# bowman-lab/enspara

Measured on AMD Instinct MI355X. Metric: frame x center RMSD pairs/sec in k-centers assign, higher is better.
Workload: dtype f32

## Files before the change

enspara_amd/csrc/ek_api_run.hip:

```cpp
#include "ek_ctx.h"
#include "ek_run_policy.h"
#include "ek_view.h"
#include <cmath>

void ek_view_free(ek_ctx *c)
{
    (void)ek_dev_free(c->v_aos);
    (void)ek_dev_free(c->v_tiles);
    (void)ek_dev_free(c->v_qtiles);
    (void)ek_dev_free(c->v_G);
    (void)ek_dev_free(c->v_dist);
    (void)ek_dev_free(c->v_assign);
    (void)ek_dev_free(c->v_act);
    (void)ek_dev_free(c->v_blockcnt);
    (void)ek_dev_free(c->v_blockoff);
    (void)ek_dev_free(c->v_count);
    c->v_aos = c->v_tiles = c->v_qtiles = nullptr;
    c->v_G = nullptr;
    c->v_dist = nullptr;
    c->v_assign = nullptr;
    c->v_act = c->v_blockcnt = c->v_blockoff = c->v_count = nullptr;
    c->view_cap = 0;
}

static int ek_view_alloc(ek_ctx *c, int64_t frames)
{
    const int64_t cap = (frames + EK_TILE - 1) / EK_TILE * EK_TILE;
    if (c->view_cap >= cap)
        return EK_OK;
    EK_HIP(ek_wait(c));
    ek_view_free(c);
    const size_t nt = (size_t)(cap / EK_TILE), A3 = (size_t)3 * c->A;
    const size_t nblk = ek_view_sel_blocks(std::max<int64_t>(c->n, 1));
    hipError_t e = hipSuccess;
#define EK_VALLOC(ptr, bytes)                                                  \
    if (e == hipSuccess)                                                       \
        e = ek_malloc_named(c, (void **)&(ptr), (bytes), #ptr);
    EK_VALLOC(c->v_aos, (size_t)cap * A3 * sizeof(float));
    EK_VALLOC(c->v_tiles, nt * A3 * EK_TILE * sizeof(float));
    EK_VALLOC(c->v_qtiles, ek_quad_tiles_bytes((int64_t)nt, c->A));
    EK_VALLOC(c->v_G, (size_t)cap * sizeof(double));
    EK_VALLOC(c->v_dist, (size_t)cap * sizeof(float));
    EK_VALLOC(c->v_assign, (size_t)cap * sizeof(int32_t));
    EK_VALLOC(c->v_act, (size_t)cap * sizeof(uint32_t));
    EK_VALLOC(c->v_blockcnt, nblk * sizeof(uint32_t));
    EK_VALLOC(c->v_blockoff, nblk * sizeof(uint32_t));
    EK_VALLOC(c->v_count, 2 * sizeof(uint32_t));
    if (e == hipSuccess)
        e = hipMemsetAsync(c->v_count, 0, 2 * sizeof(uint32_t), c->stream);
#undef EK_VALLOC
    if (e != hipSuccess) {
        (void)hipGetLastError();
        ek_view_free(c);
        if (e == hipErrorOutOfMemory) {
            c->view_nomem = true;
            return EK_ENOMEM;
        }
        EK_HIP(e);
    }
    c->view_cap = cap;
    return EK_OK;
}

struct EkViewRun {
    bool on = false;
    int64_t n = 0;
    int32_t label_lo = 0;
    double guard = 0.0;
    bool tiles_valid = false;
};

static hipError_t ek_view_poison(ek_ctx *c)
{
    const size_t cap = (size_t)c->view_cap, nt = cap / EK_TILE, A3 = (size_t)3 * c->A;
    hipError_t e = hipMemsetAsync(c->v_aos, 0xFF, cap * A3 * sizeof(float), c->stream);
    if (e == hipSuccess)
        e = hipMemsetAsync(c->v_tiles, 0xFF, nt * A3 * EK_TILE * sizeof(float), c->stream);
    if (e == hipSuccess)
        e = hipMemsetAsync(c->v_qtiles, 0xFF, ek_quad_tiles_bytes((int64_t)nt, c->A),
                           c->stream);
    if (e == hipSuccess)
        e = hipMemsetAsync(c->v_G, 0xFF, cap * sizeof(double), c->stream);
    if (e == hipSuccess)
        e = hipMemsetAsync(c->v_dist, 0xFF, cap * sizeof(float), c->stream);
    if (e == hipSuccess)
        e = hipMemsetAsync(c->v_assign, 0xFF, cap * sizeof(int32_t), c->stream);
    return e;
}

static bool ek_view_build(ek_ctx *c, int64_t n_v)
{
    ek_launch_view_build(c->v_act, n_v, c->A, c->qt_valid, c->aos, c->G, c->dist, c->assign,
                         c->v_aos, c->qt_valid ? c->v_qtiles : c->v_tiles, c->v_G, c->v_dist,
                         c->v_assign, c->stream);
    return !c->qt_valid;
}

static void ek_view_scatter_back(ek_ctx *c, EkViewRun &v)
{
    ek_launch_view_scatter(c->v_act, v.n, c->v_dist, c->v_assign, c->dist, c->assign,
                           c->hist, v.label_lo, c->hist_cap, c->ctl, c->goff, c->stream);
    v.on = false;
}

void ek_round_of(ek_ctx *c, int T, double cutoff, EkRound &R)
{
    R.dist = c->dist;
    R.assign = c->assign;
    R.vecs = c->vecs;
    R.n = c->n;
    R.n_pad = c->n_pad;
    R.goff = c->goff;
    R.A = c->A;
    R.T = T;
    R.tiles = c->tiles;
    R.qtiles = c->qtiles;
    R.aos = c->aos;
    R.G = c->G;
    R.recs = c->recsT;
    R.plan = c->plan;
    R.pend = c->pend;
    R.ord = c->ord;
    R.blockmax = c->blockmax;
    R.pm = c->pm;
    R.fm = c->fine_pick ? c->fm : nullptr;
    R.sweep = (c->pass_sweep == 2 ||
               (c->pass_sweep == 1 && ek_sweep_pays(c->n))) ? 1 : 0;
    R.top = c->top;
    R.ctile = c->ctile;
    R.ctrace = c->ctrace;
    R.hist = c->hist;
    R.ctl = c->ctl;
// ... 86 lines not shown
    if (!c->ti_tmask)
        EK_HIP(ek_dev_malloc((void **)&c->ti_tmask,
                         (size_t)std::max<int64_t>(c->n_tiles, 1) * sizeof(uint32_t)));
    return EK_OK;
}

static void ek_run_use_store(EkRun &run, bool the_view)
{
    ek_ctx *c = run.c;
    EkRound &R = run.R;
    if (the_view) {
        R.dist = c->v_dist;
        R.assign = c->v_assign;
        R.tiles = c->v_tiles;
        R.qtiles = c->v_qtiles;
        R.aos = c->v_aos;
        R.G = c->v_G;
        R.n = run.view.n;
        R.n_pad = (run.view.n + EK_TILE - 1) / EK_TILE * EK_TILE;
    } else {
        R.dist = c->dist;
        R.assign = c->assign;
        R.tiles = c->tiles;
        R.qtiles = c->qtiles;
        R.aos = c->aos;
        R.G = c->G;
        R.n = c->n;
        R.n_pad = c->n_pad;
    }
    run.nb = (int)((R.n + EK_BLOCK - 1) / EK_BLOCK);
    R.sweep = (run.fused && (c->pass_sweep == 2 ||
                             (c->pass_sweep == 1 && ek_sweep_pays(R.n)))) ? 1 : 0;
    R.cutoff = the_view ? std::max(run.dist_cutoff, run.view.guard) : run.dist_cutoff;
}

static void ek_run_leave_view(EkRun &run)
{
    if (run.pending) {
        ek_launch_round_flush(run.R, run.c->stream);
        run.pending = false;
// ... 8 lines not shown
    EkViewRun &view = run.view;
    run.looked = false;
    const EkViewPlan p =
        run.vp.decide(run.cr.last_max, run.rho, run.shrink, run.look_cnt,
                      view.on ? view.n : 0, c->n, left, run.per_round, run.forced);
    if (!p.build)
        return EK_OK;
    if (view.on) {
        ek_run_leave_view(run);
    } else if (run.pending) {
        ek_launch_round_flush(run.R, c->stream);
        run.pending = false;
    }
    uint32_t nv = 0;
    ek_launch_view_select(c->dist, c->n, p.theta, c->v_blockcnt, c->v_blockoff, c->v_act,
                          c->view_cap, c->v_count, c->stream);
    EK_CHECK_LAUNCH();
    EK_HIP(hipMemcpyAsync(&nv, c->v_count, sizeof(nv), hipMemcpyDeviceToHost, c->stream));
    EK_HIP(ek_wait(c));
    if (nv > 0 && (int64_t)nv < c->n && (int64_t)nv <= c->view_cap) {
        view.n = nv;
        view.label_lo = run.cr.n_done;
        view.guard = p.guard;
        if (run.view_mode == 3)
            EK_HIP(ek_view_poison(c));
        view.tiles_valid = ek_view_build(c, view.n);
        EK_CHECK_LAUNCH();
        view.on = true;
        ek_run_use_store(run, true);
        EK_HIP(hipMemsetAsync(c->vmask, 0, (size_t)(run.R.n_pad / EK_WAVE) * sizeof(uint32_t),
                              c->stream));
        c->view_stats[0]++;
    }
// ... 146 lines not shown
                     : ek_run_enqueue_unfused(run, form, batch);
}

static int ek_run_carry_look(EkRun &run)
{
    ek_ctx *c = run.c;
    if (!run.view_mode || run.vp.pause.tick())
        return EK_OK;
    const int64_t want_cap =
        run.forced ? c->n : (int64_t)std::ceil(run.shrink * (double)c->n);
    if (ek_view_alloc(c, want_cap) != EK_OK) {
        (void)hipGetLastError();
        run.view_mode = 0;
        return EK_OK;
    }
    EK_HIP(hipMemsetAsync(c->v_count, 0, sizeof(run.look_cnt), c->stream));
    ek_launch_view_look(run.R.dist, run.R.n, c->ctl, run.rho, EK_VIEW_REL, EK_VIEW_ABS,
                        c->v_count, c->stream);
    if (run.view.on)
        ek_launch_view_look(c->dist, c->n, c->ctl, run.rho, EK_VIEW_REL, EK_VIEW_ABS,
                            c->v_count + 1, c->stream);
    EK_CHECK_LAUNCH();
    EK_HIP(hipMemcpyAsync(run.look_cnt, c->v_count, sizeof(run.look_cnt),
                          hipMemcpyDeviceToHost, c->stream));
    run.looked = true;
    return EK_OK;
}

static int ek_run_read_back(EkRun &run, int form, int32_t &got, int32_t &ran)
{
    ek_ctx *c = run.c;
    const bool one = form == 1, masks = run.R.tmask != nullptr;
    const int32_t before = run.cr.n_done;
    EK_HIP(hipMemcpyAsync(&run.cr, c->ctl, sizeof(run.cr), hipMemcpyDeviceToHost, c->stream));
    unsigned long long ti_now[2] = {0, 0};
    if (masks)
        EK_HIP(hipMemcpyAsync(ti_now, c->ti_stats, sizeof(ti_now), hipMemcpyDeviceToHost,
                              c->stream));
// ... 281 lines not shown
}

extern "C" int ek_view_layout_check(ek_ctx *c, float theta, int64_t *out)
{
    if (!c || !out)
        return ek_fail(EK_EARG, "ek_view_layout_check: NULL argument");
    if (!c->loaded || c->n <= 0)
        return ek_fail(EK_ESTATE, "ek_view_layout_check: no frames loaded");
    EK_HIP(hipSetDevice(c->device));
    out[0] = out[1] = out[2] = out[3] = 0;
    int rc = ek_view_alloc(c, c->n);
    if (rc)
        return rc;
    uint32_t nv = 0;
    ek_launch_view_select(c->dist, c->n, theta, c->v_blockcnt, c->v_blockoff, c->v_act,
                          c->view_cap, c->v_count, c->stream);
    EK_CHECK_LAUNCH();
    EK_HIP(hipMemcpyAsync(&nv, c->v_count, sizeof(nv), hipMemcpyDeviceToHost, c->stream));
    EK_HIP(ek_wait(c));
    out[0] = nv;
    if (nv == 0 || (int64_t)nv > c->view_cap)
        return EK_OK;
    const size_t nt = ((size_t)nv + EK_TILE - 1) / EK_TILE, A3 = (size_t)3 * c->A;
    const size_t tile_words = nt * A3 * EK_TILE;
    const size_t quad_bytes = ek_quad_tiles_bytes((int64_t)nt, c->A);
    float *r_aos = nullptr, *r_tiles = nullptr, *r_qtiles = nullptr, *r_dist = nullptr;
    double *r_G = nullptr;
    int32_t *r_assign = nullptr;
    unsigned long long *diff = nullptr, got[3] = {0, 0, 0};
    hipError_t e = ek_dev_malloc((void **)&r_aos, (size_t)nv * A3 * sizeof(float));
    if (e == hipSuccess)
        e = ek_dev_malloc((void **)&r_tiles, tile_words * sizeof(float));
    if (e == hipSuccess)
        e = ek_dev_malloc((void **)&r_qtiles, quad_bytes);
    if (e == hipSuccess)
        e = ek_dev_malloc((void **)&r_G, (size_t)nv * sizeof(double));
    if (e == hipSuccess)
        e = ek_dev_malloc((void **)&r_dist, (size_t)nv * sizeof(float));
    if (e == hipSuccess)
        e = ek_dev_malloc((void **)&r_assign, (size_t)nv * sizeof(int32_t));
    if (e == hipSuccess)
        e = ek_dev_malloc((void **)&diff, sizeof(got));
    if (e == hipSuccess)
        e = hipMemsetAsync(diff, 0, sizeof(got), c->stream);
    if (e == hipSuccess)
        e = ek_view_poison(c);
    if (e == hipSuccess) {
        ek_launch_view_gather(c->v_act, nv, c->A, c->aos, c->G, c->dist, c->assign, r_aos,
                              r_tiles, r_G, r_dist, r_assign, c->stream);
        ek_launch_quad_tiles(r_tiles, (int64_t)nt, c->A, r_qtiles, c->stream);
        if (!ek_view_build(c, nv))
            ek_launch_view_tiles(c->v_qtiles, (int64_t)nt, c->A, c->v_tiles, c->stream);
        if (c->qt_valid)
            ek_launch_view_diff(c->v_qtiles, r_qtiles, quad_bytes / 4, diff, c->stream);
        ek_launch_view_diff(c->v_tiles, r_tiles, tile_words, diff + 1, c->stream);
        ek_launch_view_diff(c->v_aos, r_aos, (size_t)nv * A3, diff + 2, c->stream);
        ek_launch_view_diff(c->v_G, r_G, (size_t)nv * 2, diff + 2, c->stream);
        ek_launch_view_diff(c->v_dist, r_dist, (size_t)nv, diff + 2, c->stream);
        ek_launch_view_diff(c->v_assign, r_assign, (size_t)nv, diff + 2, c->stream);
        e = hipGetLastError();
    }
    if (e == hipSuccess)
        e = hipMemcpyAsync(got, diff, sizeof(got), hipMemcpyDeviceToHost, c->stream);
    if (e == hipSuccess)
        e = ek_wait(c);
    else
        (void)hipStreamSynchronize(c->stream);
    (void)ek_dev_free(r_aos);
    (void)ek_dev_free(r_tiles);
    (void)ek_dev_free(r_qtiles);
    (void)ek_dev_free(r_G);
    (void)ek_dev_free(r_dist);
    (void)ek_dev_free(r_assign);
    (void)ek_dev_free(diff);
    EK_HIP(e);
    out[1] = (int64_t)got[0];
    out[2] = (int64_t)got[1];
    out[3] = (int64_t)got[2];
    return EK_OK;
}

extern "C" int ek_last_run_form(ek_ctx *c, int64_t *out)
{
// ... 16 lines not shown
```

enspara_amd/csrc/ek_common.h:

```cpp
#pragma once
#include <hip/hip_runtime.h>
#include <stdint.h>
#include <stddef.h>

#include "../../include/enspara_hip.h"
#include "ek_track.h"
#include "ek_pam_limits.h"

#define EK_BLOCK 256
#define EK_WAVE 64
#define EK_MAX_ATOMS 4096

struct EkRecHdr {
    float maxdist;
    int32_t valid;
    int64_t gidx;
    double trace;
    int64_t reserved;
};
static_assert(sizeof(EkRecHdr) == 32, "record header is 32 bytes");

static inline __host__ __device__ size_t ek_rec_bytes(int A)
{
    return (sizeof(EkRecHdr) + (size_t)12 * (size_t)A + 15) & ~(size_t)15;
// ... 86 lines not shown
    uint32_t *vmask = nullptr;
    const uint32_t *tmask = nullptr;
    EkBlockMax *sweep_pm = nullptr;
    EkBlockMax *sweep_fm = nullptr;
    int sweep_nb = 0;
};
struct EkRound {
    float *dist;
    int32_t *assign;
    float *vecs;
    int64_t n, n_pad, goff;
    int A, T;
    const float *tiles;
    const float *qtiles;
    const float *aos;
    const double *G;
    unsigned char *recs;
    EkPlan *plan;
    EkPend *pend;
    EkChainOrd *ord;
    EkBlockMax *blockmax;
    EkBlockMax *pm;
    EkBlockMax *fm;
    unsigned char *top;
    float *ctile;
    double *ctrace;
    EkHist *hist;
    EkCtl *ctl;
    EkChainRow *rows;
    uint32_t *vmask;
    unsigned int *tick;
    double cutoff;
    float *ti_tab = nullptr;
    uint32_t *tmask = nullptr;
    unsigned long long *ti_stats = nullptr;
    int pick_cap = 4;
    int sweep = 0;
};
void ek_launch_round_ti(const EkRound &r, int max_labels, hipStream_t s);
void ek_launch_round_pass(const EkRound &r, hipStream_t s, bool with_order = true);
void ek_launch_round_chain(const EkRound &r, int bootstrap, hipStream_t s);
void ek_launch_round_next(const EkRound &r, int bootstrap, hipStream_t s);
void ek_launch_round_flush(const EkRound &r, hipStream_t s);

#define EK_MS_MAX_WORLD 64
#ifndef EK_MS_SLOTS
#define EK_MS_SLOTS 128
#endif
struct EkMsMsg {
    int32_t n_recs;
    int32_t cn;
    int32_t state;
    int32_t pad;
// ... 312 lines not shown
```

enspara_amd/csrc/ek_ctx.h:

```cpp
#pragma once
#include "ek_common.h"
#include "ek_pam_sparse.h"
#include "ek_pam_policy.h"

#include <stdarg.h>
#include <stdio.h>
#include <stdlib.h>
#include <string.h>

#include <algorithm>
#include <condition_variable>
#include <mutex>
#include <new>
#include <thread>
#include <vector>

void ek_msm_scratch_free(void *w);

#define EK_N_FORMS 5

int ek_set_error(int code, const char *fmt, ...);
#define ek_fail ek_set_error

#define EK_HIP(call)                                                           \
// ... 280 lines not shown
    double *ctrace = nullptr;
    int chain = 1;
    int64_t n_pad = 0;
    int32_t last_passes = 0;
    int adapt = 1;
    int64_t st_rounds[EK_N_FORMS] = {0, 0, 0, 0, 0};
    int64_t st_centers[EK_N_FORMS] = {0, 0, 0, 0, 0};
    int64_t last_form[6] = {0, 0, 0, 0, 0, 0};
    hipEvent_t evb0 = nullptr, evb1 = nullptr;

    int active_view = 1;
    int view_rho = 750;
    int view_ratio = 800;
    bool view_nomem = false;
    int64_t view_cap = 0;
    float *v_aos = nullptr, *v_tiles = nullptr, *v_qtiles = nullptr;
    double *v_G = nullptr;
    float *v_dist = nullptr;
    int32_t *v_assign = nullptr;
    uint32_t *v_act = nullptr;
    uint32_t *v_blockcnt = nullptr, *v_blockoff = nullptr;
    uint32_t *v_count = nullptr;
    int64_t view_stats[4] = {0, 0, 0, 0};

    EkMsState *ms = nullptr;
    unsigned char *ms_mbox = nullptr;
    uint32_t *ms_flags = nullptr;
    EkMsXchg ms_x;
    int ms_peers = 0;
    std::vector<void *> ms_ipc;
    int ms_T = 0;
    int ms_small = 0;
    hipEvent_t ms_ev[4] = {nullptr, nullptr, nullptr, nullptr};
    double ms_t[3] = {0.0, 0.0, 0.0};
    int64_t ms_t_n = 0;
    EkMsState ms_last;

// ... 48 lines not shown
```

enspara_amd/csrc/ek_round.hip:

```cpp
#include "ek_common.h"
#include "ek_qcp.h"
#include "ek_reduce.h"
#include "ek_chain_dev.h"
#include "ek_top_dev.h"

#ifdef EK_ROUND_STAMPS
__device__ unsigned int ek_stamp_count;
#define EK_STAMP(k) if (threadIdx.x == 0) st[k] = __builtin_amdgcn_s_memrealtime()
#else
#define EK_STAMP(k)
#endif

#define EK_ROUND_THREADS 1024

template <int NV>
__global__ void __launch_bounds__(EK_ROUND_THREADS)
ek_round_chain_kernel(EkRound r, int bootstrap)
{
    constexpr int EK_ROUND_FPT = 4;
    __shared__ float sv[EK_MAX_CANDS];
    __shared__ uint32_t si[EK_MAX_CANDS];
    __shared__ int s_napply, s_fine;
    extern __shared__ uint32_t skip[];
    const int tid = threadIdx.x;
// ... 236 lines not shown
                   64 * (v[8] / v[0]), 10 * (v[9] / v[0]), 10 * (v[10] / (v[0] / 4)),
                   10 * (v[11] / (v[12] ? v[12] : 1)), v[12]);
            for (int k = 0; k < 64 * 16; ++k)
                t[k] = 0;
        }
    }
#endif
    const EkTop *top = (const EkTop *)r.top;
    const bool done = r.ctl->stopped || r.ctl->n_done >= r.ctl->limit;
    if (!done) {
        const int lane = tid & (EK_WAVE - 1);
        const int w = blockIdx.x * (EK_BLOCK / EK_WAVE) + tid / EK_WAVE;
        const int i = w / EK_LIST_M, j = w % EK_LIST_M;
        if (i < j && j < top->n) {
            const int A = r.A;
            const float *x = r.aos + (size_t)top->idx[i] * 3 * A;
            const float *y = r.aos + (size_t)top->idx[j] * 3 * A;
            float S[9] = {0.f, 0.f, 0.f, 0.f, 0.f, 0.f, 0.f, 0.f, 0.f};
            for (int a = lane; a < A; a += EK_WAVE) {
                const float x0 = x[3 * a], x1 = x[3 * a + 1], x2 = x[3 * a + 2];
                const float y0 = y[3 * a], y1 = y[3 * a + 1], y2 = y[3 * a + 2];
                S[0] += x0 * y0; S[1] += x0 * y1; S[2] += x0 * y2;
                S[3] += x1 * y0; S[4] += x1 * y1; S[5] += x1 * y2;
                S[6] += x2 * y0; S[7] += x2 * y1; S[8] += x2 * y2;
            }
#pragma unroll
            for (int q = 0; q < 9; ++q)
#pragma unroll
                for (int off = 32; off >= 1; off >>= 1)
                    S[q] += __shfl_xor(S[q], off, 64);
            if (lane == 0) {
                const float d = ek_rmsd_from_S(S, r.G[top->idx[i]],
// ... 103 lines not shown
            plan->maxdist[tid] = sval[sel[tid]];
            plan->trace[tid] = tr;
            r.ctrace[tid] = tr;
        } else {
            h->maxdist = -__builtin_inff();
            h->valid = 0;
            h->gidx = -1;
            h->trace = 0.0;
            h->reserved = 0;
            r.ctrace[tid] = 0.0;
        }
    }
    const int A3 = 3 * r.A;
    if (T >= 16 && tid == 0)
        r.plan->n_rec = ns;
    for (int k0 = 0; T < 16 && k0 * EK_BLOCK < A3; k0 += 4) {
        float v[T][4];
#pragma unroll
        for (int c = 0; c < T; ++c) {
            const float *src = r.aos + (size_t)sidx[sel[c < ns ? c : 0]] * A3;
#pragma unroll
            for (int u = 0; u < 4; ++u) {
                const int row = tid + (k0 + u) * EK_BLOCK;
                v[c][u] = (c < ns && row < A3) ? src[row] : 0.f;
            }
        }
#pragma unroll
        for (int c = 0; c < T; ++c) {
            float *rec = (float *)(r.recs + (size_t)c * rstride + sizeof(EkRecHdr));
#pragma unroll
            for (int u = 0; u < 4; ++u) {
                const int row = tid + (k0 + u) * EK_BLOCK;
                if (row >= A3)
                    continue;
                if (c < ns)
// ... 27 lines not shown
        } else {
            plan->go = 0;
            plan->teff = 0;
            plan->used = 0;
            plan->miss = 1;
            if (!done && ns > 0)
                r.ctl->stopped = 1;
        }
    }
}

__global__ void __launch_bounds__(EK_BLOCK)
ek_round_ctile16_kernel(EkRound r, int halves)
{
    typedef float v4 __attribute__((ext_vector_type(4)));
    __shared__ uint32_t sfr[EK_MAX_CANDS];
    const EkPlan *plan = r.plan;
    const int tid = threadIdx.x;
    const int ns = plan->n_rec, go = plan->go;
    if (ns <= 0)
        return;
    if (tid < EK_MAX_CANDS)
        sfr[tid] = tid < ns ? (uint32_t)(plan->gidx[tid] - r.goff) : 0u;
    __syncthreads();
    const int A = r.A, A3 = 3 * A;
    const int n_ct = ek_ctile_atoms(A) / 16 * 3;
    const int ct_wgs = (n_ct + 3) / 4;
    if ((int)blockIdx.x < halves * ct_wgs) {
        const int half = blockIdx.x / ct_wgs;
        const int blk = (blockIdx.x % ct_wgs) * 4 + (tid >> 6), lane = tid & 63;
        if (!go || blk >= n_ct || 16 * half >= ns)
            return;
        const int S = blk / 3, k = blk % 3, kk = lane >> 4, c = 16 * half + (lane & 15);
        const float *src = r.aos + (size_t)sfr[c] * A3 + k;
        v4 v;
#pragma unroll
        for (int q = 0; q < 4; ++q) {
            const int a = 16 * S + 4 * q + kk;
            v[q] = (a < A && c < ns) ? src[3 * a] : 0.f;
        }
        *(v4 *)(r.ctile + half * ek_ctile_half_floats(A) +
                ek_ctile_index(16, 16 * S + kk, c, k)) = v;
    } else {
        const int c = blockIdx.x - halves * ct_wgs;
        if (c >= ns)
            return;
        const float *src = r.aos + (size_t)sfr[c] * A3;
        float *rec = (float *)(r.recs + (size_t)c * ek_rec_bytes(A) + sizeof(EkRecHdr));
        for (int row = tid; row < A3; row += EK_BLOCK)
            rec[row] = src[row];
    }
}

void ek_launch_round_next(const EkRound &r, int bootstrap, hipStream_t s)
{
    if (r.n <= 0)
        return;
    const unsigned blocks = (unsigned)(EK_LIST_M * EK_LIST_M / (EK_BLOCK / EK_WAVE));
    const size_t lds = (size_t)EK_LIST_M * EK_LIST_M * sizeof(float);
#define EK_NEXT_LDS(TT)                                                        \
    if (lds > 48 * 1024)                                                       \
        (void)hipFuncSetAttribute((const void *)ek_round_next_kernel<TT>,      \
// ... 84 lines not shown
}

__global__ void __launch_bounds__(EK_BLOCK)
ek_round_ti_centers_kernel(EkRound r)
{
    const EkPlan *plan = r.plan;
    if (!plan->go)
        return;
    const int lane = threadIdx.x & (EK_WAVE - 1);
    const int l = blockIdx.x * (EK_BLOCK / EK_WAVE) + threadIdx.x / EK_WAVE;
    const int k = plan->label;
    if (l >= k)
        return;
    const int A = r.A, teff = plan->teff;
    const int64_t f = r.hist[l].gidx - r.goff;
    const float *x = r.aos + (size_t)f * 3 * A;
    const double Gx = r.G[f];
    const size_t rstride = ek_rec_bytes(A);
    const int c16 = lane & 15, s = lane >> 4;
    for (int cb = 0; cb < teff; cb += 16) {
        const int c = cb + c16;
        const bool live = c < teff;
        const float *y = (const float *)(r.recs + (size_t)(live ? c : 0) * rstride +
                                         sizeof(EkRecHdr));
        float S[9] = {0.f, 0.f, 0.f, 0.f, 0.f, 0.f, 0.f, 0.f, 0.f};
        for (int a = s; a < A; a += 4) {
            const float x0 = x[3 * a], x1 = x[3 * a + 1], x2 = x[3 * a + 2];
            const float y0 = y[3 * a], y1 = y[3 * a + 1], y2 = y[3 * a + 2];
            S[0] += x0 * y0; S[1] += x0 * y1; S[2] += x0 * y2;
            S[3] += x1 * y0; S[4] += x1 * y1; S[5] += x1 * y2;
            S[6] += x2 * y0; S[7] += x2 * y1; S[8] += x2 * y2;
// ... 73 lines not shown
```

enspara_amd/csrc/ek_view.h:

```cpp
#pragma once
#include "ek_common.h"

#define EK_VIEW_SEL 1024

static inline size_t ek_view_sel_blocks(int64_t n)
{
    return (size_t)((n + EK_VIEW_SEL - 1) / EK_VIEW_SEL);
}
void ek_launch_view_select(const float *dist, int64_t n, float theta, uint32_t *blockcnt,
                           uint32_t *blockoff, uint32_t *act, int64_t act_cap,
                           uint32_t *count, hipStream_t s);
void ek_launch_view_gather(const uint32_t *act, int64_t n_v, int A, const float *aos,
                           const double *G, const float *dist, const int32_t *assign,
                           float *aos_v, float *tiles_v, double *G_v, float *dist_v,
                           int32_t *assign_v, hipStream_t s);
void ek_launch_view_build(const uint32_t *act, int64_t n_v, int A, bool quad, const float *aos,
                          const double *G, const float *dist, const int32_t *assign,
                          float *aos_v, float *out_v, double *G_v, float *dist_v,
                          int32_t *assign_v, hipStream_t s);
void ek_launch_view_tiles(const float *qtiles, int64_t n_tiles, int A, float *tiles,
                          hipStream_t s);
void ek_launch_view_look(const float *dist, int64_t n, const EkCtl *ctl, double rho, double rel,
                         double abs_, uint32_t *count, hipStream_t s);
void ek_launch_view_diff(const void *a, const void *b, size_t words,
                         unsigned long long *count, hipStream_t s);
void ek_launch_view_scatter(const uint32_t *act, int64_t n_v, const float *dist_v,
                            const int32_t *assign_v, float *dist, int32_t *assign,
                            EkHist *hist, int32_t label_lo, int32_t label_cap,
                            const EkCtl *ctl, int64_t goff, hipStream_t s);
```

enspara_amd/csrc/ek_view.hip:

```cpp
#include <algorithm>
#include "ek_view.h"

#define EK_VIEW_FPT (EK_VIEW_SEL / EK_BLOCK)
static_assert(EK_VIEW_FPT == 4, "a thread reads its frames' distances as one float4");

static __device__ __forceinline__ bool ek_view_active(float d, float theta)
{
    return !(d <= theta);
}

static __device__ __forceinline__ unsigned ek_view_flags(const float *__restrict__ dist,
                                                         int64_t f0, int64_t n, float theta)
{
    unsigned m = 0;
    if (f0 + EK_VIEW_FPT <= n) {
        const float4 t = *(const float4 *)(dist + f0);
        m = (ek_view_active(t.x, theta) ? 1u : 0u) | (ek_view_active(t.y, theta) ? 2u : 0u) |
            (ek_view_active(t.z, theta) ? 4u : 0u) | (ek_view_active(t.w, theta) ? 8u : 0u);
    } else {
        for (int q = 0; q < EK_VIEW_FPT; ++q)
            if (f0 + q < n && ek_view_active(dist[f0 + q], theta))
                m |= 1u << q;
    }
    return m;
// ... 91 lines not shown
                       theta, blockcnt);
    hipLaunchKernelGGL(ek_view_scan_kernel, dim3(1), dim3(EK_BLOCK), 0, s, blockcnt,
                       (int)nblk, act ? blockoff : (uint32_t *)nullptr, count);
    if (act)
        hipLaunchKernelGGL(ek_view_write_kernel, dim3(nblk), dim3(EK_BLOCK), 0, s, dist, n,
                           theta, blockoff, act, act_cap);
}

#define EK_VIEW_CH 16
#define EK_VIEW_ROWF (3 * EK_VIEW_CH + 1)

__global__ void __launch_bounds__(EK_BLOCK)
ek_view_gather_kernel(const uint32_t *__restrict__ act, int64_t n_v, int A,
                      const float *__restrict__ aos, const double *__restrict__ G,
                      const float *__restrict__ dist, const int32_t *__restrict__ assign,
                      float *__restrict__ aos_v, float *__restrict__ tiles_v,
                      double *__restrict__ G_v, float *__restrict__ dist_v,
                      int32_t *__restrict__ assign_v)
{
    static_assert(EK_BLOCK == EK_TILE, "one workgroup per tile of the view");
    __shared__ float stage[EK_BLOCK * EK_VIEW_ROWF];
    __shared__ uint32_t src[EK_BLOCK];
    const int t = threadIdx.x;
    const int64_t p0 = (int64_t)blockIdx.x * EK_TILE;
    const int64_t p = p0 + t;
    const bool live = p < n_v;
    const int rows_here = (int)((n_v - p0 < EK_TILE) ? (n_v - p0) : EK_TILE);
    const uint32_t f = live ? act[p] : 0u;
    src[t] = f;
    if (live) {
        G_v[p] = G[f];
        dist_v[p] = dist[f];
        assign_v[p] = assign[f];
    }
    __syncthreads();
    const size_t A3 = (size_t)3 * A;
    float *tile = tiles_v + (size_t)blockIdx.x * A3 * EK_TILE + t;
    for (int a0 = 0; a0 < A; a0 += EK_VIEW_CH) {
        const int w = 3 * ((A - a0 < EK_VIEW_CH) ? (A - a0) : EK_VIEW_CH);
        const int total = rows_here * w;
        for (int i = t; i < total; i += EK_BLOCK) {
            const int r = i / w, j = i % w;
            const float v = aos[(size_t)src[r] * A3 + 3 * a0 + j];
            stage[r * EK_VIEW_ROWF + j] = v;
            aos_v[(size_t)(p0 + r) * A3 + 3 * a0 + j] = v;
        }
        __syncthreads();
        const float *row = stage + t * EK_VIEW_ROWF;
        for (int j = 0; j < w; ++j)
            tile[(size_t)(3 * a0 + j) * EK_TILE] = live ? row[j] : 0.f;
        __syncthreads();
    }
}

void ek_launch_view_gather(const uint32_t *act, int64_t n_v, int A, const float *aos,
                           const double *G, const float *dist, const int32_t *assign,
                           float *aos_v, float *tiles_v, double *G_v, float *dist_v,
                           int32_t *assign_v, hipStream_t s)
{
    if (n_v <= 0)
        return;
    const unsigned tiles = (unsigned)((n_v + EK_TILE - 1) / EK_TILE);
    hipLaunchKernelGGL(ek_view_gather_kernel, dim3(tiles), dim3(EK_BLOCK), 0, s, act, n_v, A,
                       aos, G, dist, assign, aos_v, tiles_v, G_v, dist_v, assign_v);
}

#define EK_VIEW_BROWS 64
#define EK_VIEW_BCH 64
#define EK_VIEW_BROWF (3 * EK_VIEW_BCH + 1)
typedef float ek_view_v4f __attribute__((ext_vector_type(4)));

template <int VEC> struct EkViewVec;
template <> struct EkViewVec<4> { typedef ek_view_v4f T; };
template <> struct EkViewVec<1> { typedef float T; };

template <int VEC, bool QUAD>
__global__ void __launch_bounds__(EK_BLOCK)
ek_view_build_kernel(const uint32_t *__restrict__ act, int64_t n_v, int A,
                     const float *__restrict__ aos, const double *__restrict__ G,
                     const float *__restrict__ dist, const int32_t *__restrict__ assign,
                     float *__restrict__ aos_v, float *__restrict__ out_v,
                     double *__restrict__ G_v, float *__restrict__ dist_v,
                     int32_t *__restrict__ assign_v)
{
    static_assert(EK_BLOCK == 256 && EK_TILE == 256 && EK_WAVE == 64,
                  "four workgroups per tile of the view, one per wave of the pass");
    typedef typename EkViewVec<VEC>::T vec_t;
    constexpr int LPR = EK_VIEW_BCH / VEC;
    constexpr int RPS = EK_BLOCK / LPR;
    constexpr int SWEEPS = EK_VIEW_BROWS / RPS;
    __shared__ float stage[EK_VIEW_BROWS * EK_VIEW_BROWF];
    __shared__ uint32_t src[EK_VIEW_BROWS];
    const int t = threadIdx.x;
    const size_t tile = blockIdx.x >> 2;
    const int qw = blockIdx.x & 3;
    const int64_t p0 = (int64_t)tile * EK_TILE + EK_VIEW_BROWS * qw;
    const int rows_here =
        (int)(n_v - p0 >= EK_VIEW_BROWS ? EK_VIEW_BROWS : (n_v > p0 ? n_v - p0 : 0));
// ... 18 lines not shown
        vec_t v[SWEEPS][3];
#pragma unroll
        for (int it = 0; it < SWEEPS; ++it) {
            const int r = r0 + it * RPS;
            const vec_t *s = (const vec_t *)(aos + (size_t)src[r] * A3 + 3 * a0);
#pragma unroll
            for (int m = 0; m < 3; ++m) {
                const int j = jl + m * LPR;
                if (r < rows_here && j < we)
                    v[it][m] = s[j];
            }
        }
#pragma unroll
        for (int it = 0; it < SWEEPS; ++it) {
            const int r = r0 + it * RPS;
            vec_t *d = (vec_t *)(aos_v + (size_t)(p0 + r) * A3 + 3 * a0);
            float *st = stage + r * EK_VIEW_BROWF;
#pragma unroll
            for (int m = 0; m < 3; ++m) {
                const int j = jl + m * LPR;
                if (r < rows_here && j < we) {
                    d[j] = v[it][m];
                    if constexpr (VEC == 4) {
#pragma unroll
                        for (int x = 0; x < 4; ++x)
                            st[4 * j + x] = v[it][m][x];
                    } else {
                        st[j] = v[it][m];
                    }
                }
            }
        }
        __syncthreads();
        if constexpr (QUAD) {
            ek_view_v4f *dst = (ek_view_v4f *)out_v + tile * (size_t)NQ * 3 * EK_TILE +
                               EK_VIEW_BROWS * qw + slot;
            for (int qq = wv; qq < EK_VIEW_BCH / 4; qq += EK_BLOCK / EK_WAVE) {
// ... 13 lines not shown
                    dst[(size_t)(q * 3 + k) * EK_TILE] = o;
                }
            }
        } else {
            float *tp = out_v + tile * A3 * EK_TILE + EK_VIEW_BROWS * qw + slot;
            const float *row = stage + slot * EK_VIEW_BROWF;
            for (int j = wv; j < w; j += EK_BLOCK / EK_WAVE)
                tp[(size_t)(3 * a0 + j) * EK_TILE] = slot < rows_here ? row[j] : 0.f;
        }
        __syncthreads();
    }
}

void ek_launch_view_build(const uint32_t *act, int64_t n_v, int A, bool quad, const float *aos,
                          const double *G, const float *dist, const int32_t *assign,
                          float *aos_v, float *out_v, double *G_v, float *dist_v,
                          int32_t *assign_v, hipStream_t s)
{
    if (n_v <= 0)
        return;
    const unsigned tiles = (unsigned)((n_v + EK_TILE - 1) / EK_TILE);
#define EK_VIEW_BUILD(VEC, QUAD)                                                          \
    hipLaunchKernelGGL((ek_view_build_kernel<VEC, QUAD>), dim3(4 * tiles), dim3(EK_BLOCK), 0, \
                       s, act, n_v, A, aos, G, dist, assign, aos_v, out_v, G_v, dist_v,   \
                       assign_v)
    if (A % 4 == 0) {
        if (quad)
            EK_VIEW_BUILD(4, true);
        else
            EK_VIEW_BUILD(4, false);
    } else {
        if (quad)
            EK_VIEW_BUILD(1, true);
        else
            EK_VIEW_BUILD(1, false);
    }
#undef EK_VIEW_BUILD
}

__global__ void __launch_bounds__(EK_BLOCK)
// ... 20 lines not shown
}

void ek_launch_view_tiles(const float *qtiles, int64_t n_tiles, int A, float *tiles,
                          hipStream_t s)
{
    if (n_tiles <= 0)
        return;
    const int NQ = (A + 3) / 4;
    const unsigned gy = (unsigned)std::max<int64_t>(
        1, std::min<int64_t>(NQ, 2048 / std::max<int64_t>(n_tiles, 1)));
    hipLaunchKernelGGL(ek_view_tiles_kernel, dim3((unsigned)n_tiles, gy), dim3(EK_BLOCK), 0, s,
                       qtiles, A, NQ, tiles);
}

#define EK_VIEW_LOOK_SEL (8 * EK_VIEW_SEL)
__global__ void __launch_bounds__(EK_BLOCK)
ek_view_look_kernel(const float *__restrict__ dist, int64_t n, const EkCtl *__restrict__ ctl,
                    double rho, double rel, double abs_, uint32_t *__restrict__ count)
{
    __shared__ unsigned red[EK_BLOCK / EK_WAVE];
    const double th = (rho * (double)ctl->last_max - abs_) / (2.0 * (1.0 + rel));
    float theta = (float)th;
    if ((double)theta > th && theta > 0.f)
        theta = __uint_as_float(__float_as_uint(theta) - 1u);
    unsigned mine = 0;
#pragma unroll
    for (int q = 0; q < EK_VIEW_LOOK_SEL / EK_VIEW_SEL; ++q) {
        const int64_t f0 = (((int64_t)blockIdx.x * (EK_VIEW_LOOK_SEL / EK_VIEW_SEL) + q) *
                                EK_BLOCK + threadIdx.x) * EK_VIEW_FPT;
        mine += f0 < n ? (unsigned)__popc(ek_view_flags(dist, f0, n, theta)) : 0u;
    }
    unsigned total;
    (void)ek_view_block_scan(mine, red, &total);
    if (threadIdx.x == 0 && total)
        atomicAdd(count, total);
}

void ek_launch_view_look(const float *dist, int64_t n, const EkCtl *ctl, double rho, double rel,
                         double abs_, uint32_t *count, hipStream_t s)
{
    if (n <= 0)
        return;
    hipLaunchKernelGGL(ek_view_look_kernel,
                       dim3((unsigned)((n + EK_VIEW_LOOK_SEL - 1) / EK_VIEW_LOOK_SEL)),
                       dim3(EK_BLOCK), 0, s, dist, n, ctl, rho, rel, abs_, count);
}

__global__ void __launch_bounds__(EK_BLOCK)
ek_view_diff_kernel(const uint32_t *__restrict__ a, const uint32_t *__restrict__ b, size_t n,
                    unsigned long long *__restrict__ count)
{
    unsigned mine = 0;
    for (size_t i = (size_t)blockIdx.x * EK_BLOCK + threadIdx.x; i < n;
         i += (size_t)gridDim.x * EK_BLOCK)
        mine += a[i] != b[i] ? 1u : 0u;
    if (mine)
        atomicAdd(count, (unsigned long long)mine);
}

void ek_launch_view_diff(const void *a, const void *b, size_t words,
// ... 47 lines not shown
```

Before: 23.41 billion.

## Drop the view's AoS copy and read rows through the active index map

The compacted view no longer keeps its own copy of the AoS coordinates. Round kernels now reach the original AoS array through the view's active-index map via a new ek_round_row helper. This removes a large per-view-build write and its allocation, at the cost of an extra indirection and scattered reads when candidate rows are fetched. It also merges the two view-look kernels into one launch and double-buffers the counters by parity, which drops a memset on each look.

```diff
diff --git a/enspara_amd/csrc/ek_api_run.hip b/enspara_amd/csrc/ek_api_run.hip
--- a/enspara_amd/csrc/ek_api_run.hip
+++ b/enspara_amd/csrc/ek_api_run.hip
@@ -5,7 +5,6 @@
 
 void ek_view_free(ek_ctx *c)
 {
-    (void)ek_dev_free(c->v_aos);
     (void)ek_dev_free(c->v_tiles);
     (void)ek_dev_free(c->v_qtiles);
     (void)ek_dev_free(c->v_G);
@@ -15,11 +14,12 @@
     (void)ek_dev_free(c->v_blockcnt);
     (void)ek_dev_free(c->v_blockoff);
     (void)ek_dev_free(c->v_count);
-    c->v_aos = c->v_tiles = c->v_qtiles = nullptr;
+    (void)ek_dev_free(c->v_selcnt);
+    c->v_tiles = c->v_qtiles = nullptr;
     c->v_G = nullptr;
     c->v_dist = nullptr;
     c->v_assign = nullptr;
-    c->v_act = c->v_blockcnt = c->v_blockoff = c->v_count = nullptr;
+    c->v_act = c->v_blockcnt = c->v_blockoff = c->v_count = c->v_selcnt = nullptr;
     c->view_cap = 0;
 }
 
@@ -36,7 +36,6 @@
 #define EK_VALLOC(ptr, bytes)                                                  \
     if (e == hipSuccess)                                                       \
         e = ek_malloc_named(c, (void **)&(ptr), (bytes), #ptr);
-    EK_VALLOC(c->v_aos, (size_t)cap * A3 * sizeof(float));
     EK_VALLOC(c->v_tiles, nt * A3 * EK_TILE * sizeof(float));
     EK_VALLOC(c->v_qtiles, ek_quad_tiles_bytes((int64_t)nt, c->A));
     EK_VALLOC(c->v_G, (size_t)cap * sizeof(double));
@@ -45,9 +44,10 @@
     EK_VALLOC(c->v_act, (size_t)cap * sizeof(uint32_t));
     EK_VALLOC(c->v_blockcnt, nblk * sizeof(uint32_t));
     EK_VALLOC(c->v_blockoff, nblk * sizeof(uint32_t));
-    EK_VALLOC(c->v_count, 2 * sizeof(uint32_t));
-    if (e == hipSuccess)
-        e = hipMemsetAsync(c->v_count, 0, 2 * sizeof(uint32_t), c->stream);
+    EK_VALLOC(c->v_count, 4 * sizeof(uint32_t));
+    EK_VALLOC(c->v_selcnt, sizeof(uint32_t));
+    if (e == hipSuccess)
+        e = hipMemsetAsync(c->v_count, 0, 4 * sizeof(uint32_t), c->stream);
 #undef EK_VALLOC
     if (e != hipSuccess) {
         (void)hipGetLastError();
@@ -59,6 +59,7 @@
         EK_HIP(e);
     }
     c->view_cap = cap;
+    c->v_parity = 0;
     return EK_OK;
 }
 
@@ -73,9 +74,8 @@
 static hipError_t ek_view_poison(ek_ctx *c)
 {
     const size_t cap = (size_t)c->view_cap, nt = cap / EK_TILE, A3 = (size_t)3 * c->A;
-    hipError_t e = hipMemsetAsync(c->v_aos, 0xFF, cap * A3 * sizeof(float), c->stream);
-    if (e == hipSuccess)
-        e = hipMemsetAsync(c->v_tiles, 0xFF, nt * A3 * EK_TILE * sizeof(float), c->stream);
+    hipError_t e =
+        hipMemsetAsync(c->v_tiles, 0xFF, nt * A3 * EK_TILE * sizeof(float), c->stream);
     if (e == hipSuccess)
         e = hipMemsetAsync(c->v_qtiles, 0xFF, ek_quad_tiles_bytes((int64_t)nt, c->A),
                            c->stream);
@@ -91,8 +91,8 @@
 static bool ek_view_build(ek_ctx *c, int64_t n_v)
 {
     ek_launch_view_build(c->v_act, n_v, c->A, c->qt_valid, c->aos, c->G, c->dist, c->assign,
-                         c->v_aos, c->qt_valid ? c->v_qtiles : c->v_tiles, c->v_G, c->v_dist,
-                         c->v_assign, c->stream);
+                         c->qt_valid ? c->v_qtiles : c->v_tiles, c->v_G, c->v_dist, c->v_assign,
+                         c->stream);
     return !c->qt_valid;
 }
 
@@ -116,6 +116,7 @@
     R.tiles = c->tiles;
     R.qtiles = c->qtiles;
     R.aos = c->aos;
+    R.act = nullptr;
     R.G = c->G;
     R.recs = c->recsT;
     R.plan = c->plan;
@@ -232,7 +233,8 @@
         R.assign = c->v_assign;
         R.tiles = c->v_tiles;
         R.qtiles = c->v_qtiles;
-        R.aos = c->v_aos;
+        R.aos = c->aos;
+        R.act = c->v_act;
         R.G = c->v_G;
         R.n = run.view.n;
         R.n_pad = (run.view.n + EK_TILE - 1) / EK_TILE * EK_TILE;
@@ -242,6 +244,7 @@
         R.tiles = c->tiles;
         R.qtiles = c->qtiles;
         R.aos = c->aos;
+        R.act = nullptr;
         R.G = c->G;
         R.n = c->n;
         R.n_pad = c->n_pad;
@@ -280,9 +283,9 @@
     }
     uint32_t nv = 0;
     ek_launch_view_select(c->dist, c->n, p.theta, c->v_blockcnt, c->v_blockoff, c->v_act,
-                          c->view_cap, c->v_count, c->stream);
+                          c->view_cap, c->v_selcnt, c->stream);
     EK_CHECK_LAUNCH();
-    EK_HIP(hipMemcpyAsync(&nv, c->v_count, sizeof(nv), hipMemcpyDeviceToHost, c->stream));
+    EK_HIP(hipMemcpyAsync(&nv, c->v_selcnt, sizeof(nv), hipMemcpyDeviceToHost, c->stream));
     EK_HIP(ek_wait(c));
     if (nv > 0 && (int64_t)nv < c->n && (int64_t)nv <= c->view_cap) {
         view.n = nv;
@@ -459,14 +462,12 @@
         run.view_mode = 0;
         return EK_OK;
     }
-    EK_HIP(hipMemsetAsync(c->v_count, 0, sizeof(run.look_cnt), c->stream));
-    ek_launch_view_look(run.R.dist, run.R.n, c->ctl, run.rho, EK_VIEW_REL, EK_VIEW_ABS,
-                        c->v_count, c->stream);
-    if (run.view.on)
-        ek_launch_view_look(c->dist, c->n, c->ctl, run.rho, EK_VIEW_REL, EK_VIEW_ABS,
-                            c->v_count + 1, c->stream);
+    const int parity = c->v_parity;
+    ek_launch_view_look(run.R.dist, run.R.n, run.view.on ? c->dist : nullptr, c->n, c->ctl,
+                        run.rho, EK_VIEW_REL, EK_VIEW_ABS, c->v_count, parity, c->stream);
     EK_CHECK_LAUNCH();
-    EK_HIP(hipMemcpyAsync(run.look_cnt, c->v_count, sizeof(run.look_cnt),
+    c->v_parity = parity ^ 1;
+    EK_HIP(hipMemcpyAsync(run.look_cnt, c->v_count + 2 * parity, sizeof(run.look_cnt),
                           hipMemcpyDeviceToHost, c->stream));
     run.looked = true;
     return EK_OK;
@@ -778,9 +779,9 @@
         return rc;
     uint32_t nv = 0;
     ek_launch_view_select(c->dist, c->n, theta, c->v_blockcnt, c->v_blockoff, c->v_act,
-                          c->view_cap, c->v_count, c->stream);
+                          c->view_cap, c->v_selcnt, c->stream);
     EK_CHECK_LAUNCH();
-    EK_HIP(hipMemcpyAsync(&nv, c->v_count, sizeof(nv), hipMemcpyDeviceToHost, c->stream));
+    EK_HIP(hipMemcpyAsync(&nv, c->v_selcnt, sizeof(nv), hipMemcpyDeviceToHost, c->stream));
     EK_HIP(ek_wait(c));
     out[0] = nv;
     if (nv == 0 || (int64_t)nv > c->view_cap)
@@ -788,13 +789,11 @@
     const size_t nt = ((size_t)nv + EK_TILE - 1) / EK_TILE, A3 = (size_t)3 * c->A;
     const size_t tile_words = nt * A3 * EK_TILE;
     const size_t quad_bytes = ek_quad_tiles_bytes((int64_t)nt, c->A);
-    float *r_aos = nullptr, *r_tiles = nullptr, *r_qtiles = nullptr, *r_dist = nullptr;
+    float *r_tiles = nullptr, *r_qtiles = nullptr, *r_dist = nullptr;
     double *r_G = nullptr;
     int32_t *r_assign = nullptr;
     unsigned long long *diff = nullptr, got[3] = {0, 0, 0};
-    hipError_t e = ek_dev_malloc((void **)&r_aos, (size_t)nv * A3 * sizeof(float));
-    if (e == hipSuccess)
-        e = ek_dev_malloc((void **)&r_tiles, tile_words * sizeof(float));
+    hipError_t e = ek_dev_malloc((void **)&r_tiles, tile_words * sizeof(float));
     if (e == hipSuccess)
         e = ek_dev_malloc((void **)&r_qtiles, quad_bytes);
     if (e == hipSuccess)
@@ -810,15 +809,14 @@
     if (e == hipSuccess)
         e = ek_view_poison(c);
     if (e == hipSuccess) {
-        ek_launch_view_gather(c->v_act, nv, c->A, c->aos, c->G, c->dist, c->assign, r_aos,
-                              r_tiles, r_G, r_dist, r_assign, c->stream);
+        ek_launch_view_gather(c->v_act, nv, c->A, c->aos, c->G, c->dist, c->assign, r_tiles,
+                              r_G, r_dist, r_assign, c->stream);
         ek_launch_quad_tiles(r_tiles, (int64_t)nt, c->A, r_qtiles, c->stream);
         if (!ek_view_build(c, nv))
             ek_launch_view_tiles(c->v_qtiles, (int64_t)nt, c->A, c->v_tiles, c->stream);
         if (c->qt_valid)
             ek_launch_view_diff(c->v_qtiles, r_qtiles, quad_bytes / 4, diff, c->stream);
         ek_launch_view_diff(c->v_tiles, r_tiles, tile_words, diff + 1, c->stream);
-        ek_launch_view_diff(c->v_aos, r_aos, (size_t)nv * A3, diff + 2, c->stream);
         ek_launch_view_diff(c->v_G, r_G, (size_t)nv * 2, diff + 2, c->stream);
         ek_launch_view_diff(c->v_dist, r_dist, (size_t)nv, diff + 2, c->stream);
         ek_launch_view_diff(c->v_assign, r_assign, (size_t)nv, diff + 2, c->stream);
@@ -830,7 +828,6 @@
         e = ek_wait(c);
     else
         (void)hipStreamSynchronize(c->stream);
-    (void)ek_dev_free(r_aos);
     (void)ek_dev_free(r_tiles);
     (void)ek_dev_free(r_qtiles);
     (void)ek_dev_free(r_G);
diff --git a/enspara_amd/csrc/ek_common.h b/enspara_amd/csrc/ek_common.h
--- a/enspara_amd/csrc/ek_common.h
+++ b/enspara_amd/csrc/ek_common.h
@@ -124,6 +124,7 @@
     const float *tiles;
     const float *qtiles;
     const float *aos;
+    const uint32_t *act = nullptr;
     const double *G;
     unsigned char *recs;
     EkPlan *plan;
@@ -147,6 +148,10 @@
     int pick_cap = 4;
     int sweep = 0;
 };
+static inline __host__ __device__ const float *ek_round_row(const EkRound &r, size_t pos)
+{
+    return r.aos + (size_t)(r.act ? r.act[pos] : pos) * 3 * r.A;
+}
 void ek_launch_round_ti(const EkRound &r, int max_labels, hipStream_t s);
 void ek_launch_round_pass(const EkRound &r, hipStream_t s, bool with_order = true);
 void ek_launch_round_chain(const EkRound &r, int bootstrap, hipStream_t s);
diff --git a/enspara_amd/csrc/ek_ctx.h b/enspara_amd/csrc/ek_ctx.h
--- a/enspara_amd/csrc/ek_ctx.h
+++ b/enspara_amd/csrc/ek_ctx.h
@@ -318,13 +318,15 @@
     int view_ratio = 800;
     bool view_nomem = false;
     int64_t view_cap = 0;
-    float *v_aos = nullptr, *v_tiles = nullptr, *v_qtiles = nullptr;
+    float *v_tiles = nullptr, *v_qtiles = nullptr;
     double *v_G = nullptr;
     float *v_dist = nullptr;
     int32_t *v_assign = nullptr;
     uint32_t *v_act = nullptr;
     uint32_t *v_blockcnt = nullptr, *v_blockoff = nullptr;
     uint32_t *v_count = nullptr;
+    int v_parity = 0;
+    uint32_t *v_selcnt = nullptr;
     int64_t view_stats[4] = {0, 0, 0, 0};
 
     EkMsState *ms = nullptr;
diff --git a/enspara_amd/csrc/ek_round.hip b/enspara_amd/csrc/ek_round.hip
--- a/enspara_amd/csrc/ek_round.hip
+++ b/enspara_amd/csrc/ek_round.hip
@@ -274,8 +274,8 @@
         const int i = w / EK_LIST_M, j = w % EK_LIST_M;
         if (i < j && j < top->n) {
             const int A = r.A;
-            const float *x = r.aos + (size_t)top->idx[i] * 3 * A;
-            const float *y = r.aos + (size_t)top->idx[j] * 3 * A;
+            const float *x = ek_round_row(r, top->idx[i]);
+            const float *y = ek_round_row(r, top->idx[j]);
             float S[9] = {0.f, 0.f, 0.f, 0.f, 0.f, 0.f, 0.f, 0.f, 0.f};
             for (int a = lane; a < A; a += EK_WAVE) {
                 const float x0 = x[3 * a], x1 = x[3 * a + 1], x2 = x[3 * a + 2];
@@ -409,11 +409,17 @@
     const int A3 = 3 * r.A;
     if (T >= 16 && tid == 0)
         r.plan->n_rec = ns;
-    for (int k0 = 0; T < 16 && k0 * EK_BLOCK < A3; k0 += 4) {
+    const float *srow[T];
+    if (T < 16 && ns > 0) {
+#pragma unroll
+        for (int c = 0; c < T; ++c)
+            srow[c] = ek_round_row(r, sidx[sel[c < ns ? c : 0]]);
+    }
+    for (int k0 = 0; T < 16 && ns > 0 && k0 * EK_BLOCK < A3; k0 += 4) {
         float v[T][4];
 #pragma unroll
         for (int c = 0; c < T; ++c) {
-            const float *src = r.aos + (size_t)sidx[sel[c < ns ? c : 0]] * A3;
+            const float *src = srow[c];
 #pragma unroll
             for (int u = 0; u < 4; ++u) {
                 const int row = tid + (k0 + u) * EK_BLOCK;
@@ -471,14 +477,14 @@
 ek_round_ctile16_kernel(EkRound r, int halves)
 {
     typedef float v4 __attribute__((ext_vector_type(4)));
-    __shared__ uint32_t sfr[EK_MAX_CANDS];
+    __shared__ const float *srow[EK_MAX_CANDS];
     const EkPlan *plan = r.plan;
     const int tid = threadIdx.x;
     const int ns = plan->n_rec, go = plan->go;
     if (ns <= 0)
         return;
     if (tid < EK_MAX_CANDS)
-        sfr[tid] = tid < ns ? (uint32_t)(plan->gidx[tid] - r.goff) : 0u;
+        srow[tid] = ek_round_row(r, tid < ns ? (size_t)(plan->gidx[tid] - r.goff) : 0);
     __syncthreads();
     const int A = r.A, A3 = 3 * A;
     const int n_ct = ek_ctile_atoms(A) / 16 * 3;
@@ -489,7 +495,7 @@
         if (!go || blk >= n_ct || 16 * half >= ns)
             return;
         const int S = blk / 3, k = blk % 3, kk = lane >> 4, c = 16 * half + (lane & 15);
-        const float *src = r.aos + (size_t)sfr[c] * A3 + k;
+        const float *src = srow[c] + k;
         v4 v;
 #pragma unroll
         for (int q = 0; q < 4; ++q) {
@@ -502,7 +508,7 @@
         const int c = blockIdx.x - halves * ct_wgs;
         if (c >= ns)
             return;
-        const float *src = r.aos + (size_t)sfr[c] * A3;
+        const float *src = srow[c];
         float *rec = (float *)(r.recs + (size_t)c * ek_rec_bytes(A) + sizeof(EkRecHdr));
         for (int row = tid; row < A3; row += EK_BLOCK)
             rec[row] = src[row];
@@ -617,7 +623,7 @@
         return;
     const int A = r.A, teff = plan->teff;
     const int64_t f = r.hist[l].gidx - r.goff;
-    const float *x = r.aos + (size_t)f * 3 * A;
+    const float *x = ek_round_row(r, (size_t)f);
     const double Gx = r.G[f];
     const size_t rstride = ek_rec_bytes(A);
     const int c16 = lane & 15, s = lane >> 4;
diff --git a/enspara_amd/csrc/ek_view.h b/enspara_amd/csrc/ek_view.h
--- a/enspara_amd/csrc/ek_view.h
+++ b/enspara_amd/csrc/ek_view.h
@@ -12,16 +12,17 @@
                            uint32_t *count, hipStream_t s);
 void ek_launch_view_gather(const uint32_t *act, int64_t n_v, int A, const float *aos,
                            const double *G, const float *dist, const int32_t *assign,
-                           float *aos_v, float *tiles_v, double *G_v, float *dist_v,
-                           int32_t *assign_v, hipStream_t s);
+                           float *tiles_v, double *G_v, float *dist_v, int32_t *assign_v,
+                           hipStream_t s);
 void ek_launch_view_build(const uint32_t *act, int64_t n_v, int A, bool quad, const float *aos,
                           const double *G, const float *dist, const int32_t *assign,
-                          float *aos_v, float *out_v, double *G_v, float *dist_v,
-                          int32_t *assign_v, hipStream_t s);
+                          float *out_v, double *G_v, float *dist_v, int32_t *assign_v,
+                          hipStream_t s);
 void ek_launch_view_tiles(const float *qtiles, int64_t n_tiles, int A, float *tiles,
                           hipStream_t s);
-void ek_launch_view_look(const float *dist, int64_t n, const EkCtl *ctl, double rho, double rel,
-                         double abs_, uint32_t *count, hipStream_t s);
+void ek_launch_view_look(const float *dist, int64_t n, const float *shard_dist,
+                         int64_t shard_n, const EkCtl *ctl, double rho, double rel,
+                         double abs_, uint32_t *count, int parity, hipStream_t s);
 void ek_launch_view_diff(const void *a, const void *b, size_t words,
                          unsigned long long *count, hipStream_t s);
 void ek_launch_view_scatter(const uint32_t *act, int64_t n_v, const float *dist_v,
diff --git a/enspara_amd/csrc/ek_view.hip b/enspara_amd/csrc/ek_view.hip
--- a/enspara_amd/csrc/ek_view.hip
+++ b/enspara_amd/csrc/ek_view.hip
@@ -129,9 +129,8 @@
 ek_view_gather_kernel(const uint32_t *__restrict__ act, int64_t n_v, int A,
                       const float *__restrict__ aos, const double *__restrict__ G,
                       const float *__restrict__ dist, const int32_t *__restrict__ assign,
-                      float *__restrict__ aos_v, float *__restrict__ tiles_v,
-                      double *__restrict__ G_v, float *__restrict__ dist_v,
-                      int32_t *__restrict__ assign_v)
+                      float *__restrict__ tiles_v, double *__restrict__ G_v,
+                      float *__restrict__ dist_v, int32_t *__restrict__ assign_v)
 {
     static_assert(EK_BLOCK == EK_TILE, "one workgroup per tile of the view");
     __shared__ float stage[EK_BLOCK * EK_VIEW_ROWF];
@@ -156,9 +155,7 @@
         const int total = rows_here * w;
         for (int i = t; i < total; i += EK_BLOCK) {
             const int r = i / w, j = i % w;
-            const float v = aos[(size_t)src[r] * A3 + 3 * a0 + j];
-            stage[r * EK_VIEW_ROWF + j] = v;
-            aos_v[(size_t)(p0 + r) * A3 + 3 * a0 + j] = v;
+            stage[r * EK_VIEW_ROWF + j] = aos[(size_t)src[r] * A3 + 3 * a0 + j];
         }
         __syncthreads();
         const float *row = stage + t * EK_VIEW_ROWF;
@@ -170,14 +167,14 @@
 
 void ek_launch_view_gather(const uint32_t *act, int64_t n_v, int A, const float *aos,
                            const double *G, const float *dist, const int32_t *assign,
-                           float *aos_v, float *tiles_v, double *G_v, float *dist_v,
-                           int32_t *assign_v, hipStream_t s)
+                           float *tiles_v, double *G_v, float *dist_v, int32_t *assign_v,
+                           hipStream_t s)
 {
     if (n_v <= 0)
         return;
     const unsigned tiles = (unsigned)((n_v + EK_TILE - 1) / EK_TILE);
     hipLaunchKernelGGL(ek_view_gather_kernel, dim3(tiles), dim3(EK_BLOCK), 0, s, act, n_v, A,
-                       aos, G, dist, assign, aos_v, tiles_v, G_v, dist_v, assign_v);
+                       aos, G, dist, assign, tiles_v, G_v, dist_v, assign_v);
 }
 
 #define EK_VIEW_BROWS 64
@@ -194,9 +191,8 @@
 ek_view_build_kernel(const uint32_t *__restrict__ act, int64_t n_v, int A,
                      const float *__restrict__ aos, const double *__restrict__ G,
                      const float *__restrict__ dist, const int32_t *__restrict__ assign,
-                     float *__restrict__ aos_v, float *__restrict__ out_v,
-                     double *__restrict__ G_v, float *__restrict__ dist_v,
-                     int32_t *__restrict__ assign_v)
+                     float *__restrict__ out_v, double *__restrict__ G_v,
+                     float *__restrict__ dist_v, int32_t *__restrict__ assign_v)
 {
     static_assert(EK_BLOCK == 256 && EK_TILE == 256 && EK_WAVE == 64,
                   "four workgroups per tile of the view, one per wave of the pass");
@@ -245,13 +241,11 @@
 #pragma unroll
         for (int it = 0; it < SWEEPS; ++it) {
             const int r = r0 + it * RPS;
-            vec_t *d = (vec_t *)(aos_v + (size_t)(p0 + r) * A3 + 3 * a0);
             float *st = stage + r * EK_VIEW_BROWF;
 #pragma unroll
             for (int m = 0; m < 3; ++m) {
                 const int j = jl + m * LPR;
                 if (r < rows_here && j < we) {
-                    d[j] = v[it][m];
                     if constexpr (VEC == 4) {
 #pragma unroll
                         for (int x = 0; x < 4; ++x)
@@ -295,16 +289,15 @@
 
 void ek_launch_view_build(const uint32_t *act, int64_t n_v, int A, bool quad, const float *aos,
                           const double *G, const float *dist, const int32_t *assign,
-                          float *aos_v, float *out_v, double *G_v, float *dist_v,
-                          int32_t *assign_v, hipStream_t s)
+                          float *out_v, double *G_v, float *dist_v, int32_t *assign_v,
+                          hipStream_t s)
 {
     if (n_v <= 0)
         return;
     const unsigned tiles = (unsigned)((n_v + EK_TILE - 1) / EK_TILE);
 #define EK_VIEW_BUILD(VEC, QUAD)                                                          \
     hipLaunchKernelGGL((ek_view_build_kernel<VEC, QUAD>), dim3(4 * tiles), dim3(EK_BLOCK), 0, \
-                       s, act, n_v, A, aos, G, dist, assign, aos_v, out_v, G_v, dist_v,   \
-                       assign_v)
+                       s, act, n_v, A, aos, G, dist, assign, out_v, G_v, dist_v, assign_v)
     if (A % 4 == 0) {
         if (quad)
             EK_VIEW_BUILD(4, true);
@@ -355,11 +348,25 @@
 }
 
 #define EK_VIEW_LOOK_SEL (8 * EK_VIEW_SEL)
-__global__ void __launch_bounds__(EK_BLOCK)
-ek_view_look_kernel(const float *__restrict__ dist, int64_t n, const EkCtl *__restrict__ ctl,
-                    double rho, double rel, double abs_, uint32_t *__restrict__ count)
+static inline unsigned ek_view_look_blocks(int64_t n)
+{
+    return n > 0 ? (unsigned)((n + EK_VIEW_LOOK_SEL - 1) / EK_VIEW_LOOK_SEL) : 0u;
+}
+
+__global__ void __launch_bounds__(EK_BLOCK)
+ek_view_look_kernel(const float *__restrict__ dist_a, int64_t n_a, unsigned blocks_a,
+                    const float *__restrict__ dist_b, int64_t n_b,
+                    const EkCtl *__restrict__ ctl, double rho, double rel, double abs_,
+                    uint32_t *__restrict__ mine_cnt, uint32_t *__restrict__ other)
 {
     __shared__ unsigned red[EK_BLOCK / EK_WAVE];
+    if (blockIdx.x == 0 && threadIdx.x == 0)
+        other[0] = other[1] = 0u;
+    const bool second = blockIdx.x >= blocks_a;
+    const float *__restrict__ dist = second ? dist_b : dist_a;
+    const int64_t n = second ? n_b : n_a;
+    const int64_t blk = second ? blockIdx.x - blocks_a : blockIdx.x;
+    uint32_t *count = mine_cnt + (second ? 1 : 0);
     const double th = (rho * (double)ctl->last_max - abs_) / (2.0 * (1.0 + rel));
     float theta = (float)th;
     if ((double)theta > th && theta > 0.f)
@@ -367,8 +374,8 @@
     unsigned mine = 0;
 #pragma unroll
     for (int q = 0; q < EK_VIEW_LOOK_SEL / EK_VIEW_SEL; ++q) {
-        const int64_t f0 = (((int64_t)blockIdx.x * (EK_VIEW_LOOK_SEL / EK_VIEW_SEL) + q) *
-                                EK_BLOCK + threadIdx.x) * EK_VIEW_FPT;
+        const int64_t f0 = ((blk * (EK_VIEW_LOOK_SEL / EK_VIEW_SEL) + q) * EK_BLOCK +
+                            threadIdx.x) * EK_VIEW_FPT;
         mine += f0 < n ? (unsigned)__popc(ek_view_flags(dist, f0, n, theta)) : 0u;
     }
     unsigned total;
@@ -377,14 +384,17 @@
         atomicAdd(count, total);
 }
 
-void ek_launch_view_look(const float *dist, int64_t n, const EkCtl *ctl, double rho, double rel,
-                         double abs_, uint32_t *count, hipStream_t s)
-{
-    if (n <= 0)
-        return;
-    hipLaunchKernelGGL(ek_view_look_kernel,
-                       dim3((unsigned)((n + EK_VIEW_LOOK_SEL - 1) / EK_VIEW_LOOK_SEL)),
-                       dim3(EK_BLOCK), 0, s, dist, n, ctl, rho, rel, abs_, count);
+void ek_launch_view_look(const float *dist, int64_t n, const float *shard_dist,
+                         int64_t shard_n, const EkCtl *ctl, double rho, double rel,
+                         double abs_, uint32_t *count, int parity, hipStream_t s)
+{
+    if (!shard_dist)
+        shard_n = 0;
+    const unsigned blocks_a = std::max(1u, ek_view_look_blocks(n));
+    hipLaunchKernelGGL(ek_view_look_kernel, dim3(blocks_a + ek_view_look_blocks(shard_n)),
+                       dim3(EK_BLOCK), 0, s, dist, std::max<int64_t>(n, 0), blocks_a, shard_dist,
+                       shard_n, ctl, rho, rel, abs_, count + 2 * (parity & 1),
+                       count + 2 * ((parity & 1) ^ 1));
 }
 
 __global__ void __launch_bounds__(EK_BLOCK)
```

After: 23.97 billion, median of 6. 1.02x the previous value.
